# mfkiwl/conan-slam

Measured on AMD Instinct MI355X. Metric: ekf_update_steps_per_sec, higher is better.
Workload: dtype f32

## Files before the change

conan_slam_amd/csrc/cslam_ekf.hip:

```cpp
#include <hip/hip_runtime.h>

#include <algorithm>
#include <atomic>
#include <cfloat>
#include <cmath>
#include <cstdint>
#include <cstdlib>
#include <new>
#include <string>
#include <thread>
#include <vector>

#include "cslam_common.hpp"
#include "device_owners.hpp"
#include "ekf_kernels.hpp"
#include "ekf_kernels_fast.hpp"
#include "ekf_landmark_kernels.hpp"
#include "ekf_lookahead.hpp"
#include "ekf_pgemm_limbs.hpp"
#include "ekf_pose_kernels.hpp"
#include "host_linalg.hpp"

namespace cslam
{
__global__ void ekf_la_signal_kernel(unsigned* signal, unsigned add)
{
    if (threadIdx.x == 0)
    {
        atomicAdd(signal, add);
    }
}
__global__ void __launch_bounds__(128) ekf_la_wide_f32(LaWideArgs a)
{
    ekf_la_wide_body<1, 0>(a);
}
__global__ void __launch_bounds__(128) ekf_la_wide_f32_k64(LaWideArgs a)
{
    ekf_la_wide_body<1, 64>(a);
}
}

using namespace cslam;

namespace
{

std::atomic<int>& g_engines = ::cslam::live_engines();

constexpr int    kStagingSlots = 64;
constexpr size_t kLdsBudget    = 150 * 1024;

struct EkfBase
{
    virtual ~EkfBase() {}
    int         dtype    = CSLAM_F32;
    int         fuse_f64 = 1;
    int         pgemm_limbs_req = -1, limbs_kmin_req = -1;
    int         xcd_queues_req = -1;
    int         device   = 0;
    int         quirks   = CSLAM_Q_REF_EXACT;
    int         nmax     = 0;
    int         ncap     = 0;
    int         ldp      = 0;
    int         n        = 3;
    int         sync_mode = 1;
    int         seq_defer     = 1;
    int         lower         = 0;
    int         pipeline      = 0;
    int         pgemm_spare   = 16;
    int         gather_corr_wide = 1;
    int         pgemm_wgs     = 0;
    int         lookahead     = -1;
    Stream      stream_own, stream_b_own, stream_f_own;
    hipStream_t stream   = nullptr;
    hipStream_t stream_b = nullptr;
    long long   la_windows = 0;

    virtual int init()                                                                        = 0;
    virtual int set_state(const void* X, int n, const void* P, int ldp)                        = 0;
    virtual int get_state(void* X, void* P, int ldp)                                           = 0;
    virtual int get_x(void* X, int cap)                                                        = 0;
    virtual int get_landmarks(int first, int count, void* x, void* pll, void* pvl)             = 0;
    virtual int trace(double* tr)                                                              = 0;
    virtual int predict(double v, double swa, const void* Q, double wb, double dt)             = 0;
    virtual int update(const void* Z, int m, const void* R, const int* idf, int batch, bool on_device) = 0;
    virtual int augment(const void* Z, int q, const void* R)                                   = 0;
    virtual int observe_heading(double phi, int use)                                           = 0;
    virtual int associate(const void* Z, int m, const void* R, double g1, double g2, int* idf_out, int* kind) = 0;
    virtual int factor_status(int* flags, int clear)                                           = 0;
    virtual int set_profiling(int on)                                                          = 0;
    virtual int get_stage_times(double* ms, int* launches)                                     = 0;
    virtual int debug_last_update(void* PHT, void* S, void* G, void* W1, void* V, int* k)      = 0;
    virtual int set_deferred(int max_cols)                                                     = 0;
    virtual int do_flush()                                                                     = 0;
    virtual int resolve_predict()                                                              = 0;
    virtual void set_fuse_predict(int on)                                                      = 0;
    virtual int sync_all()                                                                     = 0;
    virtual int la_drain()                                                                     = 0;
};
// ... 264 lines not shown
            CSLAM_HIP_TRY(hipStreamSynchronize(stream_f));
        }
        inflight_mask = 0;
        return CSLAM_OK;
    }

    int wait_pgemm()
    {
        if (inflight_mask != 0 && stream_b != stream)
        {
            CSLAM_HIP_TRY(hipStreamWaitEvent(stream, ev_pgemm.get(), 0));
        }
        inflight_mask = 0;
        return CSLAM_OK;
    }

    int own_region(int r)
    {
        return (inflight_mask & (1u << r)) ? wait_pgemm() : CSLAM_OK;
    }

    int flush()
    {
        int rc = launch_pose_queue();
        if (rc)
        {
            return rc;
        }
        if (kp == 0)
        {
            return CSLAM_OK;
        }
        if ((rc = use_device()))
        {
            return rc;
        }
        T*        W   = wbase(wcur);
        const int kp8 = round_up(kp, 8);
        if (kp8 > kp && !psym4_takes(kp8))
        {
            CSLAM_HIP_TRY(hipMemset2DAsync(W + (size_t)kp * ldp, (size_t)ldp * sizeof(T), 0,
                                           (size_t)round_up(n, kTile) * sizeof(T), (size_t)(kp8 - kp), stream));
        }
        if (stream_b != stream)
        {
            CSLAM_HIP_TRY(hipEventRecord(ev_a2b.get(), stream));
            CSLAM_HIP_TRY(hipStreamWaitEvent(stream_b, ev_a2b.get(), 0));
        }
// ... 130 lines not shown
        int newm = std::max(m, 2 * mcap);
        if (int rc = la_drain())
        {
            return rc;
        }
        CSLAM_HIP_TRY(hipStreamSynchronize(stream));
        if (stream_f)
        {
            CSLAM_HIP_TRY(hipStreamSynchronize(stream_f));
        }
        PinnedBuf<unsigned char> hs;
        DevBuf<unsigned char>    ds;
        int                      rc = hs.alloc(slot_bytes(newm) * kStagingSlots);
        if (rc || (rc = ds.alloc(slot_bytes(newm) * kStagingSlots)))
        {
            return rc;
        }
        hStage = std::move(hs);
        dStage = std::move(ds);
        mcap = newm;
        return CSLAM_OK;
    }

    int stage_obs(const void* Z, const int* idf, int m, bool on_device, const T** dZ, const int** dIdf)
    {
        int rc = ensure_m(m);
        if (rc)
        {
            return rc;
        }
        int slot = stage_next;
        stage_next = (stage_next + 1) % kStagingSlots;
        if (stage_ev[slot])
        {
            CSLAM_HIP_TRY(hipEventSynchronize(stage_ev[slot].get()));
        }
        else if ((rc = stage_ev[slot].create(hipEventDisableTiming)))
        {
            return rc;
        }
        size_t         zb = (size_t)m * 2 * sizeof(T);
        unsigned char* ds = dStage.get() + slot_bytes(mcap) * slot;
        if (on_device)
        {
            hipLaunchKernelGGL(ekf_stage_obs_kernel<T>, dim3((3 * m + 255) / 256), dim3(256), 0, stream,
                               static_cast<const T*>(Z), idf, m, reinterpret_cast<T*>(ds), reinterpret_cast<int*>(ds + zb));
            CSLAM_HIP_TRY(hipGetLastError());
        }
        else
        {
            unsigned char* hs = hStage.get() + slot_bytes(mcap) * slot;
            memcpy(hs, Z, zb);
            memcpy(hs + zb, idf, (size_t)m * sizeof(int));
            CSLAM_HIP_TRY(hipMemcpyAsync(ds, hs, zb + (size_t)m * sizeof(int), hipMemcpyHostToDevice, stream));
        }
        CSLAM_HIP_TRY(hipEventRecord(stage_ev[slot].get(), stream));
        *dZ   = reinterpret_cast<const T*>(ds);
        *dIdf = reinterpret_cast<const int*>(ds + zb);
        return CSLAM_OK;
    }

    int set_state(const void* X, int nn, const void* P, int ldph) override
    {
        if (!X || !P || nn < 3 || nn > ncap || ((nn - 3) & 1) || ldph < nn)
        {
            return fail(CSLAM_ERR_BAD_ARG, "set_state: bad n=%d (cap %d) or ldp=%d", nn, ncap, ldph);
        }
        int rc = sync_all();
        if (rc)
        {
            return rc;
        }
        CSLAM_HIP_TRY(hipMemcpyAsync(dX.get(), X, (size_t)nn * sizeof(T), hipMemcpyHostToDevice, stream));
        CSLAM_HIP_TRY(hipMemcpy2DAsync(dP.get(), (size_t)ldp * sizeof(T), P, (size_t)ldph * sizeof(T),
                                       (size_t)nn * sizeof(T), (size_t)nn, hipMemcpyHostToDevice, stream));
        CSLAM_HIP_TRY(hipMemcpyAsync(dPv.get(), dP.get(), (size_t)3 * ldp * sizeof(T), hipMemcpyDeviceToDevice,
                                     stream));
        kp        = 0;
        wcur      = 0;
        last_slot = nullptr;
        hd_cols[0] = hd_cols[1] = 0;
// ... 707 lines not shown
            const int k8 = round_up(k, 8);
            if (k8 > k)
            {
                CSLAM_HIP_TRY(hipMemset2DAsync(last_slot + (size_t)k * ldp, (size_t)ldp * sizeof(T), 0,
                                               (size_t)round_up(n, kTile) * sizeof(T), (size_t)(k8 - k), stream));
            }
            if ((rc = launch_downdate(last_slot, k, stream)))
            {
                return rc;
            }
        }
        CSLAM_HIP_TRY(hipStreamSynchronize(stream));
        return CSLAM_OK;
    }


    struct LaUpd
    {
        const T*       dZ;
        const int*     dIdf;
        int            m;
        T              R[4];
        PredictArgs<T> pp;
    };
    struct FactorOut
    {
        DevBuf<T>   S, G, Gt, V, t, U, M, sub, xloc;
        DevBuf<int> idloc;
    };
    struct LaSet
    {
        Event          ev_fb;
        Event          ev_raw;
        FactorOut      fo[2];
        DevBuf<T>      XL, PvL, PH, PvLb, Dbb;
        DevBuf<T>      Y;
        DevBuf<LaModel<T>> model;
        DevBuf<unsigned>   done;
        DevBuf<long long>  stamps;
    };
    LaUpd       la_q[2];
    int         la_n = 0;
    LaSet       la;
    bool        la_ready = false;
    hipStream_t stream_f = nullptr;
    DevBuf<T>   la_WR;
    int         la_kpad  = 0;
    int         la_cus = 0;
    unsigned    la_target = 0;
    unsigned    la_seq    = 0;
    unsigned    la_sig_add = 0;
    int         la_k64 = 1;
    int         la_wg_signal = 0;

    int         la_fused   = 1;
    const T *dbgS = nullptr, *dbgGt = nullptr, *dbgV = nullptr;

    int la_ensure(int kp_cols)
    {
        constexpr int KM = 2 * kLaMaxObs;
        if (!la_ready)
        {
            int lo = 0, hi = 0;
            CSLAM_HIP_TRY(hipDeviceGetStreamPriorityRange(&lo, &hi));
            Stream sf;
            LaSet  nl;
            int    rc = sf.create_with_priority(hipStreamNonBlocking, hi);
            if (rc || (rc = nl.ev_fb.create(hipEventDisableTiming)) || (rc = nl.ev_raw.create(hipEventDisableTiming)))
            {
                return rc;
            }
            CSLAM_HIP_TRY(hipFuncSetAttribute(reinterpret_cast<const void*>(&ekf_la_chain_kernel<T, 32>),
                                              hipFuncAttributeMaxDynamicSharedMemorySize, (int)la_chain_lds<T>(32)));
            CSLAM_HIP_TRY(hipFuncSetAttribute(reinterpret_cast<const void*>(&ekf_la_chain_kernel<T, 64>),
                                              hipFuncAttributeMaxDynamicSharedMemorySize, (int)la_chain_lds<T>(64)));
            CSLAM_TRY(nl.done.alloc_zeroed_blocking(768));
            for (FactorOut& f : nl.fo)
            {
                const size_t kk = (size_t)KM * (KM + 1);
                if ((rc = f.S.alloc(kk)) || (rc = f.G.alloc(kk)) || (rc = f.Gt.alloc(kk)) || (rc = f.V.alloc(KM)) ||
                    (rc = f.t.alloc(KM)) || (rc = f.U.alloc(KM)) || (rc = f.M.alloc((size_t)3 * KM)) ||
                    (rc = f.sub.alloc((size_t)(3 + KM) * KM)) || (rc = f.xloc.alloc(3 + KM)) ||
                    (rc = f.idloc.alloc(kLaMaxObs)))
                {
                    return rc;
                }
            }
            if ((rc = nl.XL.alloc((size_t)2 * KM)) || (rc = nl.PvL.alloc((size_t)2 * KM * 3)) ||
                (rc = nl.PH.alloc((size_t)KM * KM)) || (rc = nl.PvLb.alloc((size_t)KM * 3)) ||
                (rc = nl.Dbb.alloc((size_t)KM * KM)) || (rc = nl.Y.alloc((size_t)KM * KM)) ||
                (rc = nl.model.alloc(2)) || (getenv("CSLAM_LA_STAMPS") && (rc = nl.stamps.alloc_zeroed_blocking(32))))
            {
                return rc;
            }
            if (const char* fv = getenv("CSLAM_LA_FUSED"))
            {
                la_fused = atoi(fv) ? 1 : 0;
            }
            stream_f_own = std::move(sf);
            stream_f     = stream_f_own.get();
            la           = std::move(nl);
            la_cus       = 1;
            la_target    = 0;
            la_seq       = 0;
            la_ready     = true;
        }
        if (kp_cols > la_kpad)
        {
            CSLAM_HIP_TRY(hipStreamSynchronize(stream));
            CSLAM_HIP_TRY(hipStreamSynchronize(stream_f));
            const int kpad = round_up(std::max(kp_cols, 128), 64);
            DevBuf<T> wr;
            CSLAM_TRY(wr.alloc((size_t)2 * KM * kpad));
            la_WR   = std::move(wr);
            la_kpad = kpad;
        }
        return CSLAM_OK;
    }

    bool la_eligible(int m) const
    {
// ... 2 lines not shown
        return on && !sync_mode && !pipeline && profiling != 1 && k > 16 && k <= 2 * kLaMaxObs && gather_corr_wide &&
               fuse_predict && (sizeof(T) == 4 || fuse_f64) && defer_max >= k + (la_n ? 2 * la_q[0].m : k) &&
               wcap >= k + (la_n ? 2 * la_q[0].m : k) && seq.count == 0 && hd_cols[0] == 0 && hd_cols[1] == 0 && n > 3 &&
               kp_call_limit == 0;
    }

    int la_enqueue(const T* dZ, const int* dIdf, int m, const T* R, bool on_device)
    {
        if (on_device && la_n == 0)
        {
            if (int rc = stage_obs(dZ, dIdf, m, true, &dZ, &dIdf))
            {
                return rc;
            }
        }
        LaUpd u;
        u.dZ   = dZ;
        u.dIdf = dIdf;
        u.m    = m;
        for (int i = 0; i < 4; i++)
        {
            u.R[i] = R[i];
        }
        u.pp     = pp;
        pp.valid = 0;
        la_q[la_n++] = u;
        return la_n == 2 ? la_launch_window() : CSLAM_OK;
    }

    FactorArgs<T> la_factor_args(const LaUpd& u, FactorOut& f)
    {
        FactorArgs<T> a;
        a.X   = f.xloc.get();
        a.n   = 3 + 2 * u.m;
        a.Z   = u.dZ;
        a.idf = la.fo[0].idloc.get();
        a.m   = u.m;
        for (int i = 0; i < 4; i++)
        {
            a.R[i] = u.R[i];
        }
        a.PHT      = ws.dPHT.get();
        a.ldw      = ldp;
        a.dS       = f.S.get();
        a.dG       = f.G.get();
        a.dGt      = f.Gt.get();
// ... 55 lines not shown
        {
            return rc;
        }
        pp.valid  = 0;
        fuse_now  = false;
        last_slot = slot;
        kp += k;
        dbgS      = f.S.get();
        dbgGt     = f.Gt.get();
        dbgV      = f.V.get();
        g_from_gt = true;
        sub_valid = false;
        return CSLAM_OK;
    }

    int la_launch_window()
    {
        const int nu = la_n;
        if (nu == 0)
        {
            return CSLAM_OK;
        }
        la_n = 0;
        const LaUpd ua = la_q[0], ub = la_q[1];
        const PredictArgs<T> held = pp;
        int rc = use_device();
        if (rc)
        {
            return rc;
        }
        const int ka = 2 * ua.m, kb = nu == 2 ? 2 * ub.m : 0;
        if (kp > 256 && (rc = flush()))
        {
            return rc;
        }
        if ((rc = ensure_k(2 * kLaMaxObs)) || (rc = ensure_w(ka + kb)) || (rc = la_ensure(kp)))
        {
            return rc;
        }
        if (lower && (rc = ensure_tile_list(round_up(n, kTile) / kTile)))
        {
            return rc;
        }
        const bool     safe     = g_engines.load() > 1;
        const unsigned n_blocks = (unsigned)(3 + ka + 2 * kb);
        auto launch_chain = [&]() -> int {
            LaChainArgs<T> ch;
            ch.fa   = la_factor_args(ua, la.fo[0]);
            ch.fb   = la_factor_args(nu == 2 ? ub : ua, la.fo[1]);
            ch.du_a = la.fo[0].U.get();
            ch.du_b = la.fo[1].U.get();
            ch.nu   = nu;
            ch.done = la.done.get();
            ch.target  = la_target + n_blocks;
            ch.timeout = 20000000ull;
            ch.chain_done = la.done.get() + 256;
            ch.seq        = ++la_seq;
            LaCarryArgs<T>& ca = ch.ca;
            ca.n       = n;
            ca.m_a     = ua.m;
            ca.m_b     = nu == 2 ? ub.m : 0;
            ca.idf_b   = nu == 2 ? ub.dIdf : ua.dIdf;
            ca.pp_b    = nu == 2 ? ub.pp : ua.pp;
            ca.PH      = la.PH.get();
            ca.Dbb     = la.Dbb.get();
            ca.PvLb    = la.PvLb.get();
            ca.XLb     = la.XL.get() + ka;
            ca.model_a = la.model.get();
// ... 19 lines not shown
        };
        if (!safe && (rc = launch_chain()))
        {
            return rc;
        }
        const T* Wp = wbase(wcur);
        LaRowsArgs<T> ra;
        ra.X     = dX.get();
        ra.Pv    = dPv.get();
        ra.ldp   = ldp;
        ra.n     = n;
        ra.idf_a = ua.dIdf;
        ra.ra    = ka;
        ra.idf_b = nu == 2 ? ub.dIdf : ua.dIdf;
        ra.rb    = kb;
        ra.Wp    = Wp;
        ra.ldw   = ldp;
        ra.kp    = kp;
        ra.kpad  = la_kpad;
        ra.XL    = la.XL.get();
        ra.PvL   = la.PvL.get();
        ra.WR    = la_WR.get();
        ra.flags = dFlags.get();
        hipLaunchKernelGGL(ekf_la_rows_kernel<T>, dim3(ka + kb), dim3(128), 0, stream, ra);
        LaPrepArgs<T> pa;
        pa.P       = dP.get();
        pa.ldp     = ldp;
        pa.n       = n;
        pa.lower   = lower;
        pa.X       = dX.get();
        pa.Pv      = dPv.get();
        pa.idf_a   = ua.dIdf;
        pa.idf_b   = nu == 2 ? ub.dIdf : ua.dIdf;
        pa.ra      = ka;
        pa.rb      = kb;
        pa.pp_a    = ua.pp;
        pa.XL      = la.XL.get();
        pa.PvL     = la.PvL.get();
        pa.WR      = la_WR.get();
        pa.kp      = kp;
        pa.kpad    = la_kpad;
        pa.sub_a   = la.fo[0].sub.get();
        pa.PH      = la.PH.get();
        pa.Dbb     = la.Dbb.get();
        pa.PvLb    = la.PvLb.get();
        pa.model_a = la.model.get();
        pa.xloc_a  = la.fo[0].xloc.get();
        pa.idloc   = la.fo[0].idloc.get();
        const int  k8f      = round_up(kp, 8);
        const bool pg_signal = !la_wg_signal && !safe && kp > 0 && seq.count == 0 && sizeof(T) == 4 && k8f <= 128 && lower && ldp < 32768 &&
                               !limbs_take(k8f) && stream_b == stream && hd_cols[wcur] == 0;
        pa.done    = pg_signal ? (unsigned*)nullptr : la.done.get();
        hipLaunchKernelGGL(ekf_la_blocks_kernel<T>, dim3(n_blocks), dim3(64), 0, stream, pa);
        CSLAM_HIP_TRY(hipGetLastError());
        if (safe)
        {
            CSLAM_HIP_TRY(hipEventRecord(la.ev_raw.get(), stream));
            CSLAM_HIP_TRY(hipStreamWaitEvent(stream_f, la.ev_raw.get(), 0));
            if ((rc = launch_chain()))
            {
                return rc;
            }
        }
        la_target += n_blocks;
        la_sig_add = pg_signal ? n_blocks : 0u;
        rc         = flush();
        if (la_sig_add != 0)
        {
            const unsigned add = la_sig_add;
            la_sig_add         = 0;
            hipLaunchKernelGGL(ekf_la_signal_kernel, dim3(1), dim3(64), 0, stream, la.done.get(), add);
        }
        if (rc)
        {
            return rc;
        }
        bool fused = false;
// ... 23 lines not shown
                wa.idf_a   = ua.dIdf;
                wa.idf_b   = nu == 2 ? ub.dIdf : ua.dIdf;
                wa.ma      = ua.m;
                wa.mb      = nu == 2 ? ub.m : 0;
                wa.valid_a = ua.pp.valid;
                wa.valid_b = nu == 2 ? ub.pp.valid : 0;
                wa.w_a     = ua.pp.w;
                wa.w_b     = nu == 2 ? ub.pp.w : 0;
                wa.model_a = la.model.get();
                wa.model_b = la.model.get() + 1;
                wa.Gt_a    = la.fo[0].Gt.get();
                wa.u_a     = la.fo[0].U.get();
                wa.M_a     = la.fo[0].M.get();
                wa.sub_a   = la.fo[0].sub.get();
                wa.Gt_b    = la.fo[1].Gt.get();
                wa.u_b     = la.fo[1].U.get();
                wa.M_b     = la.fo[1].M.get();
                wa.sub_b   = la.fo[1].sub.get();
                wa.Y_b     = la.Y.get();
                wa.W1a     = wbase(wcur) + (size_t)kp * ldp;
                wa.W1b     = wa.W1a + (size_t)ka * ldp;
                wa.ldw     = ldp;
                wa.wv_out  = ws.dWv.get();
                if (la_k64 && ua.m == 32 && (nu == 1 || ub.m == 32))
                {
                    hipLaunchKernelGGL(ekf_la_wide_f32_k64, dim3(round_up(n, kTile) / 32), dim3(128), 0, stream, wa);
                }
                else
                {
                    hipLaunchKernelGGL(ekf_la_wide_f32, dim3(round_up(n, kTile) / 32), dim3(128), 0, stream, wa);
                }
                CSLAM_HIP_TRY(hipGetLastError());
                last_slot = nullptr;
                last_k    = 0;
                kp += ka + kb;
                sub_valid = false;
            }
        }
        if (!fused && ((rc = la_wide(ua, la.fo[0], la.ev_fb.get())) || (nu == 2 && (rc = la_wide(ub, la.fo[1],
                                                                                                 nullptr)))))
        {
            return rc;
        }
        pp = held;
        la_windows++;
        if (la.stamps.get() && la_windows == 300)
        {
            long long h[32];
            CSLAM_HIP_TRY(hipStreamSynchronize(stream));
            CSLAM_HIP_TRY(hipMemcpy(h, la.stamps.get(), sizeof(h), hipMemcpyDeviceToHost));
            fprintf(stderr, "[cslam la wide stamps, 10 ns ticks] ids+columns issue:%lld poll+DMA wait:%lld pht_a:%lld gain_a:%lld store+share W1_a:%lld pht_b+corr:%lld share+G_b:%lld gain_b:%lld store_b:%lld\n",
                    h[17] - h[16], h[18] - h[17], h[19] - h[18], h[20] - h[19], h[21] - h[20], h[22] - h[21], h[23] - h[22],
                    h[24] - h[23], h[25] - h[24]);
            fprintf(stderr, "[cslam la stamps, cycles] load+observe:%lld sums:%lld symmetrise:%lld cholesky:%lld (first half %lld) inverse:%lld outputs:%lld total:%lld\n",
                    h[6] - h[0], h[7] - h[6], h[1] - h[7], h[2] - h[1], h[5] ? h[5] - h[1] : 0, h[3] - h[2], h[4] - h[3], h[4] - h[0]);
        }
        return CSLAM_OK;
    }

    int la_drain() override { return la_n ? la_launch_window() : CSLAM_OK; }

    int update(const void* Zv, int m, const void* Rv, const int* idf, int batch, bool on_device) override
    {
        if (m < 0 || !Rv || (m > 0 && (!Zv || !idf)))
        {
            return fail(CSLAM_ERR_BAD_ARG, "update: bad arguments (m=%d)", m);
        }
        if (m == 0)
        {
            return CSLAM_OK;
        }
        int rc = use_device();
        if (rc)
        {
            return rc;
        }
        const T*   R    = static_cast<const T*>(Rv);
        const T*   dZ   = static_cast<const T*>(Zv);
        const int* dIdf = idf;
        if (!on_device)
        {
            const int nf = (n - 3) / 2;
            for (int i = 0; i < m; i++)
// ... 749 lines not shown

int cslam_ekf_set_pgemm_workgroups(cslam_ekf_t h, int workgroups)
{
    CSLAM_NEED(h);
    if (workgroups < 0)
    {
        return fail(CSLAM_ERR_BAD_ARG, "set_pgemm_workgroups: negative");
    }
    B(h)->pgemm_wgs = workgroups;
    return CSLAM_OK;
}

int cslam_ekf_lookahead_windows(cslam_ekf_t h, long long* windows)
{
    CSLAM_NEED(h);
    if (!windows)
    {
        return fail(CSLAM_ERR_BAD_ARG, "lookahead_windows: null");
    }
    *windows = B(h)->la_windows;
    return CSLAM_OK;
}

int cslam_ekf_get_streams(cslam_ekf_t h, void** chain_stream, void** pgemm_stream)
{
    CSLAM_NEED(h);
    if (chain_stream)
    {
        *chain_stream = reinterpret_cast<void*>(B(h)->stream);
    }
    if (pgemm_stream)
    {
        *pgemm_stream = reinterpret_cast<void*>(B(h)->stream_b);
    }
    return CSLAM_OK;
}

int cslam_ekf_run_many(cslam_ekf_t* handles, int count, int steps, const double* v, const double* swa, const void* Q,
                       double wb, double dt, const void* const* dZ, const int* const* d_idf, int m, const void* R,
                       int batch)
{
    if (!handles || count < 0 || steps < 0 || m < 0 || !R || !Q || (steps > 0 && (!v || !swa)) || (m > 0 && (!dZ || !d_idf)))
    {
        return fail(CSLAM_ERR_BAD_ARG, "run_many: bad arguments");
    }
    for (int i = 0; i < count; i++)
// ... 98 lines not shown
```

conan_slam_amd/csrc/ekf_lookahead.hpp:

```cpp
#pragma once

#include <hip/hip_runtime.h>

#include "ekf_kernels.hpp"
#include "ekf_kernels_fast.hpp"

namespace cslam
{

constexpr int kLaMaxObs = 32;

__device__ inline int la_row(const int* __restrict__ idf, int s, int n)
{
    return 3 + 2 * clamp_idf(idf[s >> 1], n) - 2 + (s & 1);
}

template <typename T>
struct LaRowsArgs
{
    const T* X;
    const T* Pv;
    int      ldp, n;
    const int* idf_a;
    int        ra;
// ... 110 lines not shown
template <typename T>
struct LaPrepArgs
{
    const T* P;
    int      ldp, n, lower;
    const T* X;
    const T* Pv;
    const int* idf_a;
    const int* idf_b;
    int ra, rb;
    PredictArgs<T> pp_a;
    const T *XL, *PvL, *WR;
    int kp, kpad;
    T* sub_a;
    T* PH;
    T* Dbb;
    T* PvLb;
    LaModel<T>* model_a;
    T*   xloc_a;
    int* idloc;
    unsigned* done;
};

template <typename T>
__device__ __forceinline__ void ekf_la_blocks_body(const LaPrepArgs<T>& a)
{
    __shared__ T wrow[256];
    __shared__ T s_xl[3 + 2 * kLaMaxObs];
    __shared__ T s_coef[kLaMaxObs * 10];
    __shared__ T s_pvv[9], s_g[2], s_e3[3];
    __shared__ T s_d[2 * kLaMaxObs];
    __shared__ T s_e[2 * kLaMaxObs * 3];
    const int tid = threadIdx.x;
    const int ra = a.ra, rb = a.rb, ma = ra >> 1;
    int       b    = blockIdx.x;
    int       type = 0, s = b;
    if (b >= 3)
    {
        b -= 3;
        type = (b < ra) ? 1 : ((b < ra + rb) ? 2 : 3);
        s    = (type == 1) ? b : ((type == 2) ? b - ra : b - ra - rb);
    }
    const int* idf_r = (type <= 1) ? a.idf_a : a.idf_b;
    const int* idf_c = (type == 3) ? a.idf_b : a.idf_a;
    const int  nc    = (type == 3) ? rb : ra;
    const int  wr_r  = (type <= 1) ? s : ra + s;
    const int  wr_c0 = (type == 3) ? ra : 0;
    int        row   = 0;
    T          pcell = (T)0;
    T          e3[3] = {(T)0, (T)0, (T)0};
    if (type != 0)
    {
        row = la_row(idf_r, s, a.n);
        for (int q = tid; q < a.kp; q += 64)
        {
            wrow[q] = a.WR[(size_t)q * 128 + wr_r];
        }
        if (tid < nc)
        {
            pcell = p_sym<T>(a.P, a.ldp, row, la_row(idf_c, tid, a.n), a.lower);
        }
        if (tid == 0)
        {
            e3[0] = a.PvL[wr_r * 3 + 0], e3[1] = a.PvL[wr_r * 3 + 1], e3[2] = a.PvL[wr_r * 3 + 2];
        }
    }
    T ee[3] = {(T)0, (T)0, (T)0};
    int erow = 0;
    if (type == 0 && tid < ra)
    {
        ee[0] = a.PvL[tid * 3 + 0], ee[1] = a.PvL[tid * 3 + 1], ee[2] = a.PvL[tid * 3 + 2];
        erow  = la_row(a.idf_a, tid, a.n);
    }
    if (tid < ra)
    {
        s_xl[3 + tid] = a.XL[tid];
    }
    if (tid == 0)
    {
        T pose_in[3] = {a.X[0], a.X[1], a.X[2]}, pvv_in[9], pose[3], g[2], pvv[9];
        for (int e = 0; e < 9; e++)
        {
            pvv_in[e] = a.Pv[(size_t)(e / 3) * a.ldp + (e % 3)];
// ... 111 lines not shown
            out[2 * tid + 1] = v1;
        }
        if (type == 2 && tid < 3)
        {
            a.PvLb[s * 3 + tid] = s_e3[tid];
        }
    }
    if (a.done == nullptr)
    {
        return;
    }
    __builtin_amdgcn_fence(__ATOMIC_RELEASE, "agent");
    __syncthreads();
    if (tid == 0)
    {
        atomicAdd(a.done + 16 * (blockIdx.x & 15u), 1u);
    }
}

template <typename T>
__global__ void __launch_bounds__(64) ekf_la_blocks_kernel(LaPrepArgs<T> a)
{
    ekf_la_blocks_body<T>(a);
}

template <typename T>
struct LaCarryArgs
{
    int n, m_a, m_b;
    const int* idf_b;
    PredictArgs<T> pp_b;
    const T *PH, *Dbb, *PvLb, *XLb;
    const LaModel<T>* model_a;
    const T *Gt_a, *u_a, *M_a, *sub_a;
    T*          sub_b;
    T*          xloc_b;
    LaModel<T>* model_b;
    T*          Y_b;
};

template <typename T>
inline size_t la_carry_lds()
{
    constexpr int KM = 2 * kLaMaxObs, LD = KM + 4, LB = 3 + KM + 1;
    return ((size_t)KM * LD + (size_t)(3 + KM) * LB + kLaMaxObs * 10 + (3 + KM) + 4 * KM + 3 * KM) * sizeof(T) + 64;
}
// ... 389 lines not shown
{
    const float* P;
    int          ldp, n, lower;
    float*       X;
    float*       Pv;
    int          nu;
    const int *  idf_a, *idf_b;
    int          ma, mb;
    int          valid_a, valid_b, w_a, w_b;
    const LaModel<float>*model_a, *model_b;
    const float *Gt_a, *u_a, *M_a, *sub_a;
    const float *Gt_b, *u_b, *M_b, *sub_b, *Y_b;
    float *      W1a, *W1b;
    int          ldw;
    float*       wv_out;
    const unsigned* chain_done;
    unsigned        seq;
    unsigned long long timeout;
    int*            flags;
    long long*      stamps;
    long long*      wg_times;
};

__device__ __forceinline__ int la_q_of(int t, int r, int lh)
{
    return 32 * t + (r & 3) + 8 * (r >> 2) + 4 * lh;
}

template <int PAIRS = 1, int KFIX = 0>
__device__ __forceinline__ void ekf_la_wide_body(const LaWideArgs& a)
{
    __shared__ __attribute__((aligned(16))) float s_G[2][4 * 1024];
    __shared__ __attribute__((aligned(16))) float s_Y[4 * 1024];
    __shared__ __attribute__((aligned(16))) float s_model[2][512];
    __shared__ __attribute__((aligned(16))) float s_u[2][256];
    __shared__ __attribute__((aligned(16))) float s_M[2][256];
    __shared__ int   s_fx[2][kLaMaxObs];
    __shared__ float s_sum_all[PAIRS][4][32];
    const int tid = threadIdx.x, wave = __builtin_amdgcn_readfirstlane(tid >> 6), lane = tid & 63, lj = lane & 31, lh = lane >> 5;
    const int wv = wave & 1, pr = wave >> 1;
    float (*s_sum)[32] = s_sum_all[pr];
    const int row0 = (blockIdx.x * PAIRS + pr) * 32;
    const int row  = row0 + lj;
    const int rowc = row < a.n ? row : a.n - 1;
    const int ka = KFIX ? KFIX : 2 * a.ma, kb = KFIX ? KFIX : 2 * a.mb;
    int       stamp_i = 0;
    auto      stamp   = [&]() {
        if (a.stamps != nullptr && blockIdx.x == (gridDim.x >> 1) && tid == 0)
        {
            a.stamps[stamp_i++] = (long long)__builtin_amdgcn_s_memrealtime();
        }
    };
    stamp();
    if constexpr (PAIRS == 2)
    {
        if (a.wg_times != nullptr && tid == 0)
        {
            a.wg_times[2 * blockIdx.x] = (long long)__builtin_amdgcn_s_memrealtime();
        }
    }
    const int id_a = lane < a.ma ? a.idf_a[lane] : 1;
    const int id_b = (a.nu == 2 && lane < a.mb) ? a.idf_b[lane] : 1;
    float pv0 = a.Pv[(size_t)0 * a.ldp + rowc], pv1 = a.Pv[(size_t)1 * a.ldp + rowc], pv2 = a.Pv[(size_t)2 * a.ldp + rowc];
    float x   = a.X[rowc];
    if (tid < kLaMaxObs)
    {
        s_fx[0][tid] = 3 + 2 * clamp_idf(id_a, a.n) - 2;
        s_fx[1][tid] = 3 + 2 * clamp_idf(id_b, a.n) - 2;
    }
    __syncthreads();
    float pcol[2][16];
    {
        int fxv[2][8];
#pragma unroll
        for (int ub = 0; ub < 2; ub++)
        {
#pragma unroll
            for (int i = 0; i < 8; i++)
            {
                const int o = (32 * wv + (2 * i & 3) + 8 * (2 * i >> 2) + 4 * lh) >> 1;
                fxv[ub][i]  = s_fx[ub][o < kLaMaxObs ? o : 0];
            }
        }
#pragma unroll
        for (int ub = 0; ub < 2; ub++)
        {
            const int k = ub == 0 ? ka : kb;
#pragma unroll
            for (int i = 0; i < 8; i++)
            {
                const int  q  = 32 * wv + (2 * i & 3) + 8 * (2 * i >> 2) + 4 * lh;
                const bool in = q < k && (ub == 0 || a.nu == 2);
                const int  fx = in ? fxv[ub][i] : 3;
// ... 144 lines not shown
    };
    auto store_w1 = [&](float* W, int k, bool last) {
#pragma unroll
        for (int r = 0; r < 16; r++)
        {
            const int c = la_q_of(wv, r, lh);
            if (c < k)
            {
                if (row < 3)
                {
                    if (last)
                    {
                        a.wv_out[(size_t)row * k + c] = w1[r];
                    }
                    W[(size_t)c * a.ldw + row] = 0.f;
                }
                else
                {
                    W[(size_t)c * a.ldw + row] = w1[r];
                }
            }
        }
    };
    using U0 = std::integral_constant<int, 0>;
    using U1 = std::integral_constant<int, 1>;

    if (a.valid_a && row >= 3 && row - 3 < a.w_a)
    {
        float o0, o1, o2;
        predict_stripe_col<float>(s_model[0][0], s_model[0][1], pv0, pv1, pv2, &o0, &o1, &o2);
        pv0 = o0, pv1 = o1, pv2 = o2;
    }
    build_own(U0{}, ka, a.sub_a);
    share();
    stamp();
    gain(U0{}, ka);
    stamp();
    store_w1(a.W1a, ka, a.nu == 1);
    const float* pred_last = s_model[0];
    if (a.nu == 2)
    {
        __syncthreads();
#pragma unroll
        for (int r = 0; r < 16; r++)
        {
            own[r] = (row >= 3) ? w1[r] : 0.f;
        }
        share();
        const float xs = s_sum[0][lj], xm0 = s_sum[1][lj], xm1 = s_sum[2][lj], xm2 = s_sum[3][lj];
        if (row >= 3)
        {
            x += xs;
            pv0 -= xm0, pv1 -= xm1, pv2 -= xm2;
        }
        stamp();
        if (a.valid_b && row >= 3 && row - 3 < a.w_b)
        {
            float o0, o1, o2;
            predict_stripe_col<float>(s_model[1][0], s_model[1][1], pv0, pv1, pv2, &o0, &o1, &o2);
            pv0 = o0, pv1 = o1, pv2 = o2;
        }
// ... 24 lines not shown
                    c0 = __builtin_amdgcn_mfma_f32_32x32x2f32(y[i], full[i], c0, 0, 0, 0);
                }
            }
            if (row >= 3)
            {
#pragma unroll
                for (int r = 0; r < 16; r++)
                {
                    own[r] -= c0[r] + c1[r];
                }
            }
        }
        stamp();
        __syncthreads();
        dma(a.Gt_b, kb * kb, s_G[1]);
        xch = s_G[0] + pr * 2048;
        share();
        __builtin_amdgcn_s_waitcnt(0x0F70);
        __syncthreads();
        stamp();
        gain(U1{}, kb);
        stamp();
        store_w1(a.W1b, kb, true);
        pred_last = s_model[1];
    }
    __syncthreads();
    stamp();
    if constexpr (PAIRS == 2)
    {
        if (a.wg_times != nullptr && tid == 0)
        {
            a.wg_times[2 * blockIdx.x + 1] = (long long)__builtin_amdgcn_s_memrealtime();
        }
    }
    if (wv == 0 && lh == 0 && row < a.n)
    {
        const float xs = s_sum[0][lj], xm0 = s_sum[1][lj], xm1 = s_sum[2][lj], xm2 = s_sum[3][lj];
        if (row >= 3)
        {
            a.X[row]                        = x + xs;
            a.Pv[(size_t)0 * a.ldp + row] = pv0 - xm0;
            a.Pv[(size_t)1 * a.ldp + row] = pv1 - xm1;
            a.Pv[(size_t)2 * a.ldp + row] = pv2 - xm2;
        }
        else
        {
            const int   r     = row;
            const float av[3] = {pred_last[5 + r], pred_last[5 + r + 3], pred_last[5 + r + 6]};
            const float dv[3] = {xm0, xm1, xm2};
            a.X[r]            = pred_last[2 + r] + xs;
#pragma unroll
            for (int c = 0; c < 3; c++)
            {
                if (c == r)
                {
                    a.Pv[(size_t)c * a.ldp + r] = av[c] - dv[c];
                }
                else if (c < r)
                {
                    const float bcr             = pred_last[5 + c + 3 * r];
                    a.Pv[(size_t)c * a.ldp + r] = av[c] - dv[c];
                    a.Pv[(size_t)r * a.ldp + c] = bcr - dv[c];
                }
            }
        }
    }
// ... 222 lines not shown
```

conan_slam_amd/ekf.py:

```python
from __future__ import annotations

import ctypes as C

import numpy as np

from . import _capi
from ._capi import (F32, F64, Q_REF_EXACT, Q_TEXTBOOK, check)


def _vp(a: np.ndarray):
    return a.ctypes.data_as(C.c_void_p)


class EKF:
    def __init__(self, max_landmarks: int, dtype=np.float32, device: int = -1, quirks: int = Q_REF_EXACT,
                 sync_mode: bool = True):
        self.dtype = np.dtype(dtype)
        if self.dtype not in (np.dtype(np.float32), np.dtype(np.float64)):
            raise ValueError("dtype must be float32 or float64")
        self._L = _capi.lib()
        self._h = C.c_void_p(None)
        code = F32 if self.dtype == np.float32 else F64
        check(self._L.cslam_ekf_create(C.c_int(max_landmarks), C.c_int(code), C.c_int(device), C.c_int(quirks),
                                       C.byref(self._h)))
# ... 61 lines not shown
    def get_x(self):
        n = self.n
        X = np.zeros(n, dtype=self.dtype)
        check(self._L.cslam_ekf_get_x(self._h, _vp(X), C.c_int(n)))
        return X

    def get_p(self):
        return self.get_state()[1]

    X = property(get_x)
    P = property(get_p)

    def trace(self) -> float:
        t = C.c_double(0.0)
        check(self._L.cslam_ekf_trace(self._h, C.byref(t)))
        return t.value

    def synchronize(self):
        check(self._L.cslam_ekf_synchronize(self._h))

    def lookahead_windows(self) -> int:
        w = C.c_longlong(0)
        check(self._L.cslam_ekf_lookahead_windows(self._h, C.byref(w)))
        return w.value

    def landmarks(self, first: int = 1, count: int = None):
        if count is None:
            count = max((self.n - 3) // 2 - first + 1, 0)
        x = np.empty((count, 2), dtype=self.dtype)
        pll = np.empty((count, 4), dtype=self.dtype)
        pvl = np.empty((count, 6), dtype=self.dtype)
        check(self._L.cslam_ekf_get_landmarks(self._h, int(first), int(count), _vp(x), _vp(pll), _vp(pvl)))
        return x, pll.reshape(count, 2, 2).transpose(0, 2, 1).copy(), pvl.reshape(count, 2, 3).transpose(0, 2, 1).copy()

    def factor_status(self, clear: bool = False) -> int:
        f = C.c_int(0)
        check(self._L.cslam_ekf_factor_status(self._h, C.byref(f), C.c_int(1 if clear else 0)))
        return f.value

    def predict(self, v, swa, Q, wb, dt):
        Q = self._mat22(Q)
        check(self._L.cslam_ekf_predict(self._h, C.c_double(float(v)), C.c_double(float(swa)), _vp(Q),
                                        C.c_double(float(wb)), C.c_double(float(dt))))

    def update(self, Z, R, idf, batch: bool = False):
        Z = np.asarray(Z, dtype=self.dtype)
# ... 231 lines not shown
```

include/cslam.h:

```cpp
#ifndef CSLAM_H
#define CSLAM_H

#ifdef __cplusplus
extern "C" {
#endif

#define CSLAM_VERSION 100

#define CSLAM_OK 0
#define CSLAM_ERR_BAD_ARG 1
#define CSLAM_ERR_CAPACITY 2
#define CSLAM_ERR_HIP 3
#define CSLAM_ERR_NO_DEVICE 4
#define CSLAM_ERR_ALLOC 5
#define CSLAM_FACTOR_OK 0
#define CSLAM_FACTOR_FALLBACK 1
#define CSLAM_FACTOR_ZEROED 2
#define CSLAM_FACTOR_SKIPPED 4
#define CSLAM_FACTOR_INTERNAL 16
#define CSLAM_FACTOR_BAD_IDF 8
#define CSLAM_FACTOR_HEADING_SKIPPED 32

#define CSLAM_F32 0
#define CSLAM_F64 1
// ... 29 lines not shown
int cslam_ekf_trace(cslam_ekf_t h, double* trace);
int cslam_ekf_synchronize(cslam_ekf_t h);
int cslam_ekf_factor_status(cslam_ekf_t h, int* flags, int clear);

int cslam_ekf_predict(cslam_ekf_t h, double v, double swa, const void* Q, double wb, double dt);

int cslam_ekf_update(cslam_ekf_t h, const void* Z, int m, const void* R, const int* idf, int batch);

int cslam_ekf_update_device(cslam_ekf_t h, const void* dZ, int m, const void* R, const int* d_idf, int batch);

int cslam_ekf_augment(cslam_ekf_t h, const void* Z, int q, const void* R);

int cslam_ekf_observe_heading(cslam_ekf_t h, double phi, int use_heading);

int cslam_ekf_associate(cslam_ekf_t h, const void* Z, int m, const void* R, double gate1, double gate2, int* idf_out,
                        int* kind_out);

int cslam_ekf_set_deferred(cslam_ekf_t h, int max_pending_columns);
int cslam_ekf_flush(cslam_ekf_t h);

int cslam_ekf_get_streams(cslam_ekf_t h, void** chain_stream, void** pgemm_stream);

int cslam_ekf_lookahead_windows(cslam_ekf_t h, long long* windows);

int cslam_ekf_set_pgemm_workgroups(cslam_ekf_t h, int workgroups);

int cslam_ekf_run_many(cslam_ekf_t* handles, int count, int steps, const double* v, const double* swa, const void* Q,
                       double wb, double dt, const void* const* dZ, const int* const* d_idf, int m, const void* R,
                       int batch);

typedef struct cslam_ekf_batch* cslam_ekf_batch_t;
int cslam_ekf_batch_create(int instances, int n_landmarks, int device, int quirks, cslam_ekf_batch_t* out);
int cslam_ekf_batch_destroy(cslam_ekf_batch_t h);
int cslam_ekf_batch_set_state(cslam_ekf_batch_t h, int instance, const float* X, int n, const float* P, int ldp);
int cslam_ekf_batch_get_state(cslam_ekf_batch_t h, int instance, float* X, float* P, int ldp);
int cslam_ekf_batch_run(cslam_ekf_batch_t h, int steps, const double* v, const double* swa, const float* Q, double wb,
                        double dt, const float* const* dZ, const int* const* d_idf, int m, const float* R);
int cslam_ekf_batch_flush(cslam_ekf_batch_t h);
int cslam_ekf_batch_synchronize(cslam_ekf_batch_t h);
int cslam_ekf_batch_trace(cslam_ekf_batch_t h, double* traces );
int cslam_ekf_batch_factor_status(cslam_ekf_batch_t h, int* flags );
int cslam_ekf_batch_info(cslam_ekf_batch_t h, int* instances, int* n, long long* windows);
int cslam_ekf_batch_set_profiling(cslam_ekf_batch_t h, int every);
int cslam_ekf_batch_get_pgemm_time(cslam_ekf_batch_t h, double* ms_sum, int* launches);

int cslam_ekf_batch_create_capacity(int instances, int max_landmarks, int n_landmarks, int device, int quirks,
// ... 93 lines not shown
```

Before: 13220.

## Defer wide update kernel and fuse next window's row gather into it

The lookahead path now holds back the wide gain/update kernel of one window so it can be launched together with the next window's prep work. Extra blocks in that kernel gather the next window's P entries into a raw buffer, check for bad landmark ids, and snapshot the observations. The wide blocks also hand off the W1 rows, X and Pv values the next window needs. This removes the separate rows kernel and a launch per window, and lets the blocks kernel read the pre-gathered cells. In exchange the code adds cross-block ordering assumptions inside one kernel (relaxed atomic loads of rows being written) and many eligibility conditions that fall back to the old launch sequence.

```diff
diff --git a/conan_slam_amd/csrc/cslam_ekf.hip b/conan_slam_amd/csrc/cslam_ekf.hip
--- a/conan_slam_amd/csrc/cslam_ekf.hip
+++ b/conan_slam_amd/csrc/cslam_ekf.hip
@@ -37,6 +37,14 @@
 __global__ void __launch_bounds__(128) ekf_la_wide_f32_k64(LaWideArgs a)
 {
     ekf_la_wide_body<1, 64>(a);
+}
+__global__ void __launch_bounds__(128) ekf_la_wide_f32_next(LaWideArgs a, LaWideNext nx)
+{
+    ekf_la_wide_body<1, 0, true>(a, &nx);
+}
+__global__ void __launch_bounds__(128) ekf_la_wide_f32_k64_next(LaWideArgs a, LaWideNext nx)
+{
+    ekf_la_wide_body<1, 64, true>(a, &nx);
 }
 }
 
@@ -75,6 +83,7 @@
     hipStream_t stream   = nullptr;
     hipStream_t stream_b = nullptr;
     long long   la_windows = 0;
+    long long   la_held_windows = 0;
 
     virtual int init()                                                                        = 0;
     virtual int set_state(const void* X, int n, const void* P, int ldp)                        = 0;
@@ -385,8 +394,8 @@
 
     int flush()
     {
-        int rc = launch_pose_queue();
-        if (rc)
+        int rc = la_submit_held(nullptr);
+        if (rc || (rc = launch_pose_queue()))
         {
             return rc;
         }
@@ -563,7 +572,8 @@
         return CSLAM_OK;
     }
 
-    int stage_obs(const void* Z, const int* idf, int m, bool on_device, const T** dZ, const int** dIdf)
+    int stage_obs(const void* Z, const int* idf, int m, bool on_device, const T** dZ, const int** dIdf, bool copy = true,
+                  int* slot_out = nullptr)
     {
         int rc = ensure_m(m);
         if (rc)
@@ -582,6 +592,16 @@
         }
         size_t         zb = (size_t)m * 2 * sizeof(T);
         unsigned char* ds = dStage.get() + slot_bytes(mcap) * slot;
+        if (slot_out)
+        {
+            *slot_out = slot;
+        }
+        *dZ   = reinterpret_cast<const T*>(ds);
+        *dIdf = reinterpret_cast<const int*>(ds + zb);
+        if (on_device && !copy)
+        {
+            return CSLAM_OK;
+        }
         if (on_device)
         {
             hipLaunchKernelGGL(ekf_stage_obs_kernel<T>, dim3((3 * m + 255) / 256), dim3(256), 0, stream,
@@ -596,8 +616,6 @@
             CSLAM_HIP_TRY(hipMemcpyAsync(ds, hs, zb + (size_t)m * sizeof(int), hipMemcpyHostToDevice, stream));
         }
         CSLAM_HIP_TRY(hipEventRecord(stage_ev[slot].get(), stream));
-        *dZ   = reinterpret_cast<const T*>(ds);
-        *dIdf = reinterpret_cast<const int*>(ds + zb);
         return CSLAM_OK;
     }
 
@@ -1351,6 +1369,7 @@
         int            m;
         T              R[4];
         PredictArgs<T> pp;
+        bool           dev;
     };
     struct FactorOut
     {
@@ -1361,6 +1380,7 @@
     {
         Event          ev_fb;
         Event          ev_raw;
+        DevBuf<T>      Praw;
         FactorOut      fo[2];
         DevBuf<T>      XL, PvL, PH, PvLb, Dbb;
         DevBuf<T>      Y;
@@ -1382,6 +1402,14 @@
     int         la_k64 = 1;
     int         la_wg_signal = 0;
 
+    struct LaHeld
+    {
+        bool       on = false;
+        LaWideArgs wa;
+        int        k64, grid, ka, kb, kp0;
+    };
+    LaHeld      la_held;
+    int         la_held_enable = 1;
     int         la_fused   = 1;
     const T *dbgS = nullptr, *dbgGt = nullptr, *dbgV = nullptr;
 
@@ -1395,7 +1423,8 @@
             Stream sf;
             LaSet  nl;
             int    rc = sf.create_with_priority(hipStreamNonBlocking, hi);
-            if (rc || (rc = nl.ev_fb.create(hipEventDisableTiming)) || (rc = nl.ev_raw.create(hipEventDisableTiming)))
+            if (rc || (rc = nl.ev_fb.create(hipEventDisableTiming)) || (rc = nl.ev_raw.create(hipEventDisableTiming)) ||
+                (rc = nl.Praw.alloc((size_t)2 * 3 * KM * 64)))
             {
                 return rc;
             }
@@ -1426,6 +1455,10 @@
             {
                 la_fused = atoi(fv) ? 1 : 0;
             }
+            if (const char* hv = getenv("CSLAM_LA_HELD"))
+            {
+                la_held_enable = atoi(hv) ? 1 : 0;
+            }
             stream_f_own = std::move(sf);
             stream_f     = stream_f_own.get();
             la           = std::move(nl);
@@ -1474,6 +1507,7 @@
         {
             u.R[i] = R[i];
         }
+        u.dev    = on_device && la_n == 1;
         u.pp     = pp;
         pp.valid = 0;
         la_q[la_n++] = u;
@@ -1575,7 +1609,8 @@
             return CSLAM_OK;
         }
         la_n = 0;
-        const LaUpd ua = la_q[0], ub = la_q[1];
+        const LaUpd ua = la_q[0];
+        LaUpd       ub = la_q[1];
         const PredictArgs<T> held = pp;
         int rc = use_device();
         if (rc)
@@ -1597,6 +1632,29 @@
         }
         const bool     safe     = g_engines.load() > 1;
         const unsigned n_blocks = (unsigned)(3 + ka + 2 * kb);
+        bool hold = false, carry = false;
+        if constexpr (std::is_same<T, float>::value)
+        {
+            hold  = la_fused && la_held_enable && nu == 2 && !safe;
+            carry = hold && la_held.on && la_held.kp0 == 0 && kp == la_held.ka + la_held.kb && kp <= la_kpad &&
+                    seq.count == 0 && lower && ldp < 32768 && stream_b == stream && hd_cols[wcur] == 0 &&
+                    !limbs_take(round_up(kp, 8));
+        }
+        if (!carry && (rc = la_submit_held(nullptr)))
+        {
+            return rc;
+        }
+        const T*   src_Z     = nullptr;
+        const int* src_idf_b = ub.dIdf;
+        int        snap_slot = -1;
+        if (hold && ub.dev)
+        {
+            src_Z = ub.dZ;
+            if ((rc = stage_obs(src_Z, src_idf_b, ub.m, true, &ub.dZ, &ub.dIdf, !carry, &snap_slot)))
+            {
+                return rc;
+            }
+        }
         auto launch_chain = [&]() -> int {
             LaChainArgs<T> ch;
             ch.fa   = la_factor_args(ua, la.fo[0]);
@@ -1662,7 +1720,6 @@
         ra.PvL   = la.PvL.get();
         ra.WR    = la_WR.get();
         ra.flags = dFlags.get();
-        hipLaunchKernelGGL(ekf_la_rows_kernel<T>, dim3(ka + kb), dim3(128), 0, stream, ra);
         LaPrepArgs<T> pa;
         pa.P       = dP.get();
         pa.ldp     = ldp;
@@ -1691,8 +1748,40 @@
         const bool pg_signal = !la_wg_signal && !safe && kp > 0 && seq.count == 0 && sizeof(T) == 4 && k8f <= 128 && lower && ldp < 32768 &&
                                !limbs_take(k8f) && stream_b == stream && hd_cols[wcur] == 0;
         pa.done    = pg_signal ? (unsigned*)nullptr : la.done.get();
-        hipLaunchKernelGGL(ekf_la_blocks_kernel<T>, dim3(n_blocks), dim3(64), 0, stream, pa);
-        CSLAM_HIP_TRY(hipGetLastError());
+        if (carry)
+        {
+            if constexpr (std::is_same<T, float>::value)
+            {
+                LaWideNext nx;
+                nx.idf_a       = ua.dIdf;
+                nx.idf_b       = src_idf_b;
+                nx.ra          = ka;
+                nx.rb          = kb;
+                nx.XL          = la.XL.get();
+                nx.PvL         = la.PvL.get();
+                nx.WR          = la_WR.get();
+                nx.Praw        = la.Praw.get() + (size_t)(la_seq & 1u) * 3 * 2 * kLaMaxObs * 64;
+                nx.wide_blocks = la_held.grid;
+                nx.snap_Z      = src_Z;
+                nx.snap_Zout   = const_cast<T*>(ub.dZ);
+                nx.snap_idf    = const_cast<int*>(ub.dIdf);
+                if ((rc = la_submit_held(&nx)))
+                {
+                    return rc;
+                }
+                (void)snap_slot;
+                hipLaunchKernelGGL(ekf_la_blocks_raw_kernel<T>, dim3(n_blocks), dim3(64), 0, stream, pa,
+                                   (const T*)nx.Praw);
+                CSLAM_HIP_TRY(hipGetLastError());
+                la_held_windows++;
+            }
+        }
+        else
+        {
+            hipLaunchKernelGGL(ekf_la_rows_kernel<T>, dim3(ka + kb), dim3(128), 0, stream, ra);
+            hipLaunchKernelGGL(ekf_la_blocks_kernel<T>, dim3(n_blocks), dim3(64), 0, stream, pa);
+            CSLAM_HIP_TRY(hipGetLastError());
+        }
         if (safe)
         {
             CSLAM_HIP_TRY(hipEventRecord(la.ev_raw.get(), stream));
@@ -1762,15 +1851,17 @@
                 wa.W1b     = wa.W1a + (size_t)ka * ldp;
                 wa.ldw     = ldp;
                 wa.wv_out  = ws.dWv.get();
-                if (la_k64 && ua.m == 32 && (nu == 1 || ub.m == 32))
+                la_held.on   = true;
+                la_held.wa   = wa;
+                la_held.k64  = (la_k64 && ua.m == 32 && (nu == 1 || ub.m == 32)) ? 1 : 0;
+                la_held.grid = round_up(n, kTile) / 32;
+                la_held.ka   = ka;
+                la_held.kb   = kb;
+                la_held.kp0  = kp;
+                if (!hold && (rc = la_submit_held(nullptr)))
                 {
-                    hipLaunchKernelGGL(ekf_la_wide_f32_k64, dim3(round_up(n, kTile) / 32), dim3(128), 0, stream, wa);
+                    return rc;
                 }
-                else
-                {
-                    hipLaunchKernelGGL(ekf_la_wide_f32, dim3(round_up(n, kTile) / 32), dim3(128), 0, stream, wa);
-                }
-                CSLAM_HIP_TRY(hipGetLastError());
                 last_slot = nullptr;
                 last_k    = 0;
                 kp += ka + kb;
@@ -1798,7 +1889,47 @@
         return CSLAM_OK;
     }
 
-    int la_drain() override { return la_n ? la_launch_window() : CSLAM_OK; }
+    int la_drain() override
+    {
+        const int rc = la_n ? la_launch_window() : CSLAM_OK;
+        return rc ? rc : la_submit_held(nullptr);
+    }
+
+    int la_submit_held(const LaWideNext* nx)
+    {
+        if (!la_held.on)
+        {
+            return CSLAM_OK;
+        }
+        la_held.on = false;
+        if (int rc = use_device())
+        {
+            return rc;
+        }
+        const LaWideArgs& wa = la_held.wa;
+        if (nx != nullptr)
+        {
+            const dim3 grid(la_held.grid + (nx->ra + 2 * nx->rb + 7) / 8);
+            if (la_held.k64)
+            {
+                hipLaunchKernelGGL(ekf_la_wide_f32_k64_next, grid, dim3(128), 0, stream, wa, *nx);
+            }
+            else
+            {
+                hipLaunchKernelGGL(ekf_la_wide_f32_next, grid, dim3(128), 0, stream, wa, *nx);
+            }
+        }
+        else if (la_held.k64)
+        {
+            hipLaunchKernelGGL(ekf_la_wide_f32_k64, dim3(la_held.grid), dim3(128), 0, stream, wa);
+        }
+        else
+        {
+            hipLaunchKernelGGL(ekf_la_wide_f32, dim3(la_held.grid), dim3(128), 0, stream, wa);
+        }
+        CSLAM_HIP_TRY(hipGetLastError());
+        return CSLAM_OK;
+    }
 
     int update(const void* Zv, int m, const void* Rv, const int* idf, int batch, bool on_device) override
     {
@@ -2594,6 +2725,17 @@
     return CSLAM_OK;
 }
 
+int cslam_ekf_lookahead_held_windows(cslam_ekf_t h, long long* windows)
+{
+    CSLAM_NEED(h);
+    if (!windows)
+    {
+        return fail(CSLAM_ERR_BAD_ARG, "lookahead_held_windows: null");
+    }
+    *windows = B(h)->la_held_windows;
+    return CSLAM_OK;
+}
+
 int cslam_ekf_get_streams(cslam_ekf_t h, void** chain_stream, void** pgemm_stream)
 {
     CSLAM_NEED(h);
diff --git a/conan_slam_amd/csrc/ekf_lookahead.hpp b/conan_slam_amd/csrc/ekf_lookahead.hpp
--- a/conan_slam_amd/csrc/ekf_lookahead.hpp
+++ b/conan_slam_amd/csrc/ekf_lookahead.hpp
@@ -156,8 +156,8 @@
     unsigned* done;
 };
 
-template <typename T>
-__device__ __forceinline__ void ekf_la_blocks_body(const LaPrepArgs<T>& a)
+template <typename T, bool RAW = false>
+__device__ __forceinline__ void ekf_la_blocks_body(const LaPrepArgs<T>& a, const T* __restrict__ praw = nullptr)
 {
     __shared__ T wrow[256];
     __shared__ T s_xl[3 + 2 * kLaMaxObs];
@@ -192,7 +192,14 @@
         }
         if (tid < nc)
         {
-            pcell = p_sym<T>(a.P, a.ldp, row, la_row(idf_c, tid, a.n), a.lower);
+            if constexpr (RAW)
+            {
+                pcell = praw[(size_t)(blockIdx.x - 3) * 64 + tid];
+            }
+            else
+            {
+                pcell = p_sym<T>(a.P, a.ldp, row, la_row(idf_c, tid, a.n), a.lower);
+            }
         }
         if (tid == 0)
         {
@@ -350,6 +357,12 @@
 __global__ void __launch_bounds__(64) ekf_la_blocks_kernel(LaPrepArgs<T> a)
 {
     ekf_la_blocks_body<T>(a);
+}
+
+template <typename T>
+__global__ void __launch_bounds__(64) ekf_la_blocks_raw_kernel(LaPrepArgs<T> a, const T* praw)
+{
+    ekf_la_blocks_body<T, true>(a, praw);
 }
 
 template <typename T>
@@ -785,14 +798,27 @@
     long long*      wg_times;
 };
 
+struct LaWideNext
+{
+    const int *idf_a, *idf_b;
+    int        ra, rb;
+    float *    XL, *PvL, *WR;
+    float*     Praw;
+    int        wide_blocks;
+    const float* snap_Z;
+    float*       snap_Zout;
+    int*         snap_idf;
+};
+
 __device__ __forceinline__ int la_q_of(int t, int r, int lh)
 {
     return 32 * t + (r & 3) + 8 * (r >> 2) + 4 * lh;
 }
 
-template <int PAIRS = 1, int KFIX = 0>
-__device__ __forceinline__ void ekf_la_wide_body(const LaWideArgs& a)
-{
+template <int PAIRS = 1, int KFIX = 0, bool NEXT = false>
+__device__ __forceinline__ void ekf_la_wide_body(const LaWideArgs& a, const LaWideNext* nxp = nullptr)
+{
+    static_assert(!NEXT || PAIRS == 1, "the next-window block belongs to the single filter's kernel");
     __shared__ __attribute__((aligned(16))) float s_G[2][4 * 1024];
     __shared__ __attribute__((aligned(16))) float s_Y[4 * 1024];
     __shared__ __attribute__((aligned(16))) float s_model[2][512];
@@ -800,8 +826,62 @@
     __shared__ __attribute__((aligned(16))) float s_M[2][256];
     __shared__ int   s_fx[2][kLaMaxObs];
     __shared__ float s_sum_all[PAIRS][4][32];
+    __shared__ int   s_hit[NEXT ? 129 : 1];
     const int tid = threadIdx.x, wave = __builtin_amdgcn_readfirstlane(tid >> 6), lane = tid & 63, lj = lane & 31, lh = lane >> 5;
     const int wv = wave & 1, pr = wave >> 1;
+    if constexpr (NEXT)
+    {
+        const LaWideNext& nx = *nxp;
+        if ((int)blockIdx.x >= nx.wide_blocks)
+        {
+            const int ra = nx.ra, rb = nx.rb, col = tid & 63;
+#pragma unroll
+            for (int i = 0; i < 4; i++)
+            {
+                const int b = ((int)blockIdx.x - nx.wide_blocks) * 8 + (tid >> 6) * 4 + i;
+                if (b < ra + 2 * rb)
+                {
+                    const int  type  = (b < ra) ? 1 : ((b < ra + rb) ? 2 : 3);
+                    const int  s     = (type == 1) ? b : ((type == 2) ? b - ra : b - ra - rb);
+                    const int* idf_r = (type == 1) ? nx.idf_a : nx.idf_b;
+                    const int* idf_c = (type == 3) ? nx.idf_b : nx.idf_a;
+                    const int  nc    = (type == 3) ? rb : ra;
+                    if (col < nc)
+                    {
+                        nx.Praw[(size_t)b * 64 + col] =
+                            p_sym<float>(a.P, a.ldp, la_row(idf_r, s, a.n), la_row(idf_c, col, a.n), a.lower);
+                    }
+                }
+            }
+            if ((int)blockIdx.x == nx.wide_blocks)
+            {
+                if (tid < ((ra + rb) >> 1))
+                {
+                    const int id = (tid < (ra >> 1)) ? nx.idf_a[tid] : nx.idf_b[tid - (ra >> 1)];
+                    if (id < 1 || id > ((a.n - 3) >> 1))
+                    {
+                        atomicOr(&a.flags[0], kFlagBadIdf);
+                    }
+                }
+                if (nx.snap_Z != nullptr)
+                {
+                    if (tid < rb)
+                    {
+                        nx.snap_Zout[tid] = nx.snap_Z[tid];
+                    }
+                    if (tid < (rb >> 1))
+                    {
+                        nx.snap_idf[tid] = nx.idf_b[tid];
+                    }
+                }
+            }
+            return;
+        }
+        if (tid == 0)
+        {
+            s_hit[0] = 0;
+        }
+    }
     float (*s_sum)[32] = s_sum_all[pr];
     const int row0 = (blockIdx.x * PAIRS + pr) * 32;
     const int row  = row0 + lj;
@@ -832,6 +912,18 @@
         s_fx[1][tid] = 3 + 2 * clamp_idf(id_b, a.n) - 2;
     }
     __syncthreads();
+    if constexpr (NEXT)
+    {
+        const LaWideNext& nx = *nxp;
+        if (tid < nx.ra + nx.rb)
+        {
+            const int r = (tid < nx.ra) ? la_row(nx.idf_a, tid, a.n) : la_row(nx.idf_b, tid - nx.ra, a.n);
+            if (r >= row0 && r < row0 + 32)
+            {
+                s_hit[1 + atomicAdd(&s_hit[0], 1)] = ((r - row0) << 8) | tid;
+            }
+        }
+    }
     float pcol[2][16];
     {
         int fxv[2][8];
@@ -1022,6 +1114,28 @@
             }
         }
     };
+    auto hand_w1 = [&](int q0, int k) {
+        if constexpr (NEXT)
+        {
+            const int nh = s_hit[0];
+            for (int h = 0; h < nh; h++)
+            {
+                const int e = s_hit[1 + h];
+                if ((e >> 8) == lj)
+                {
+#pragma unroll
+                    for (int r = 0; r < 16; r++)
+                    {
+                        const int c = la_q_of(wv, r, lh);
+                        if (c < k)
+                        {
+                            nxp->WR[(size_t)(q0 + c) * 128 + (e & 255)] = w1[r];
+                        }
+                    }
+                }
+            }
+        }
+    };
     using U0 = std::integral_constant<int, 0>;
     using U1 = std::integral_constant<int, 1>;
 
@@ -1037,6 +1151,7 @@
     gain(U0{}, ka);
     stamp();
     store_w1(a.W1a, ka, a.nu == 1);
+    hand_w1(0, ka);
     const float* pred_last = s_model[0];
     if (a.nu == 2)
     {
@@ -1107,6 +1222,7 @@
         gain(U1{}, kb);
         stamp();
         store_w1(a.W1b, kb, true);
+        hand_w1(ka, kb);
         pred_last = s_model[1];
     }
     __syncthreads();
@@ -1127,6 +1243,25 @@
             a.Pv[(size_t)0 * a.ldp + row] = pv0 - xm0;
             a.Pv[(size_t)1 * a.ldp + row] = pv1 - xm1;
             a.Pv[(size_t)2 * a.ldp + row] = pv2 - xm2;
+            if constexpr (NEXT)
+            {
+                const int nh = s_hit[0];
+                for (int h = 0; h < nh; h++)
+                {
+                    const int e = s_hit[1 + h];
+                    if ((e >> 8) == lj)
+                    {
+                        const int slot       = e & 255;
+                        nxp->XL[slot]          = __hip_atomic_load(&a.X[row], __ATOMIC_RELAXED, __HIP_MEMORY_SCOPE_AGENT);
+#pragma unroll
+                        for (int c = 0; c < 3; c++)
+                        {
+                            nxp->PvL[slot * 3 + c] =
+                                __hip_atomic_load(&a.Pv[(size_t)c * a.ldp + row], __ATOMIC_RELAXED, __HIP_MEMORY_SCOPE_AGENT);
+                        }
+                    }
+                }
+            }
         }
         else
         {
diff --git a/conan_slam_amd/ekf.py b/conan_slam_amd/ekf.py
--- a/conan_slam_amd/ekf.py
+++ b/conan_slam_amd/ekf.py
@@ -107,6 +107,11 @@
     def lookahead_windows(self) -> int:
         w = C.c_longlong(0)
         check(self._L.cslam_ekf_lookahead_windows(self._h, C.byref(w)))
+        return w.value
+
+    def lookahead_held_windows(self) -> int:
+        w = C.c_longlong(0)
+        check(self._L.cslam_ekf_lookahead_held_windows(self._h, C.byref(w)))
         return w.value
 
     def landmarks(self, first: int = 1, count: int = None):
diff --git a/include/cslam.h b/include/cslam.h
--- a/include/cslam.h
+++ b/include/cslam.h
@@ -75,6 +75,7 @@
 int cslam_ekf_get_streams(cslam_ekf_t h, void** chain_stream, void** pgemm_stream);
 
 int cslam_ekf_lookahead_windows(cslam_ekf_t h, long long* windows);
+int cslam_ekf_lookahead_held_windows(cslam_ekf_t h, long long* windows);
 
 int cslam_ekf_set_pgemm_workgroups(cslam_ekf_t h, int workgroups);
 
```

Measured after the change: 13220 (median of 2 runs). No clear change (-0.0%).
